# DeepMed-Lab-ECNU/BCP

Hardware: AMD Instinct MI355X
Metric: training volumes/sec (LA 112x112x80 V-Net, BCP self-training step) (higher is better)
Workload: dtype f32 (fp16x2 split operands); 1 GPU; LA 3D V-Net BCP self-train step, per-GPU batch 4 (2 labeled), 112x112x80 patches, SGD m0.9 wd1e-4, EMA 0.99 (BASELINE.json configs[1]); global_batch=4, parallelism=dp1

## Files before the change

### bcp_amd/csrc/api.hip

```cpp
#include "common.h"
#include "../../include/bcp_hip.h"
#include <cstring>

namespace bcp {
static thread_local char g_err[512] = "";
void set_error(const char* fmt, ...) {
  va_list ap;
  va_start(ap, fmt);
  vsnprintf(g_err, sizeof(g_err), fmt, ap);
  va_end(ap);
}
Options& options() {
  static Options o;
  return o;
}
}

extern "C" int bcp_version(void) { return BCP_ABI_VERSION; }

extern "C" int bcp_set_option(const char* name, const char* value) {
  BCP_REQUIRE(name && value, "bcp_set_option: null argument");
  bcp::Options& o = bcp::options();
  const bcp::Options def;
  long long v[5] = {0, 0, 0, 0, 0};
  const int n = sscanf(value, "%lld,%lld,%lld,%lld,%lld", &v[0], &v[1], &v[2], &v[3], &v[4]);
  const bool reset = n <= 0;
#define BCP_OPT_INT(field) if (!strcmp(name, #field)) { o.field = reset ? def.field : (int)v[0]; return BCP_OK; }
  BCP_OPT_INT(conv3_p) BCP_OPT_INT(splitk) BCP_OPT_INT(conv3_b6_flat_sk) BCP_OPT_INT(conv3_b6_cfg2d) BCP_OPT_INT(conv3_b6_w22) BCP_OPT_INT(conv3_b6_pipe) BCP_OPT_INT(conv3_b6_cin16max) BCP_OPT_INT(res_pcu) BCP_OPT_INT(res_nt) BCP_OPT_INT(wgrad_nt)
  BCP_OPT_INT(tn_groups) BCP_OPT_INT(cc_tile) BCP_OPT_INT(pack_sections) BCP_OPT_INT(cc_select_blocks) BCP_OPT_INT(conv3_b6) BCP_OPT_INT(conv3_b6_levels) BCP_OPT_INT(conv3_b6_direct) BCP_OPT_INT(conv3_b6_flat) BCP_OPT_INT(conv3_b6_minvox) BCP_OPT_INT(wgrad_b6) BCP_OPT_INT(wgrad_b6_minvox) BCP_OPT_INT(wgrad_b6_levels) BCP_OPT_INT(wgrad_b6_slots) BCP_OPT_INT(cc_border_dedupe) BCP_OPT_INT(cc_count_tile) BCP_OPT_INT(cc_fuse_select) BCP_OPT_INT(gemm_walk) BCP_OPT_INT(gemm_pipe) BCP_OPT_INT(gemm_stat_r) BCP_OPT_INT(norm_apply_cap) BCP_OPT_INT(norm_apply_vec) BCP_OPT_INT(k2_stats) BCP_OPT_INT(k2_bwd_stats) BCP_OPT_INT(up_recompute) BCP_OPT_INT(wgrad_b6_deep) BCP_OPT_INT(wgrad_b6_deep_nt) BCP_OPT_INT(wgrad_b6_deep_slots) BCP_OPT_INT(wgrad_b6_deep_tile) BCP_OPT_INT(norm_slabs) BCP_OPT_INT(conv3_f16) BCP_OPT_INT(fuse_bwd_stats) BCP_OPT_INT(conv3_xcd) BCP_OPT_INT(mix_c1) BCP_OPT_INT(whatif) BCP_OPT_INT(c3d16_form) BCP_OPT_INT(norm_own) BCP_OPT_INT(wgrad_reduce_flat) BCP_OPT_INT(norm_fin_rows) BCP_OPT_INT(norm_fuse_fin)
#undef BCP_OPT_INT
  if (!strcmp(name, "conv3_sk_elems")) { o.conv3_sk_elems = reset ? def.conv3_sk_elems : v[0]; return BCP_OK; }
  if (!strcmp(name, "res_tile2d_vox")) { o.res_tile2d_vox = reset ? def.res_tile2d_vox : v[0]; return BCP_OK; }
  if (!strcmp(name, "conv3_cfg")) {
    BCP_REQUIRE(reset || n == 4, "bcp_set_option: conv3_cfg wants TD,TH,TW,NT");
    for (int i = 0; i < 4; ++i) o.conv3_cfg[i] = reset ? 0 : (int)v[i];
    return BCP_OK;
  }
  if (!strcmp(name, "wgrad_tile")) {
    BCP_REQUIRE(reset || n >= 3, "bcp_set_option: wgrad_tile wants TD,TH,TW[,min_voxels,max_voxels]");
    for (int i = 0; i < 5; ++i) o.wgrad_tile[i] = def.wgrad_tile[i];
    for (int i = 0; i < n && !reset; ++i) o.wgrad_tile[i] = v[i];
    return BCP_OK;
  }
  bcp::set_error("bcp_set_option: unknown option '%s'", name);
  return BCP_EINVAL;
}
extern "C" const char* bcp_last_error(void) { return bcp::g_err; }

extern "C" int bcp_device_arch(char* buf, int n) {
  BCP_REQUIRE(buf && n > 0, "bcp_device_arch: bad buffer");
  int dev = 0;
  hipDeviceProp_t prop;
  if (hipGetDevice(&dev) != hipSuccess || hipGetDeviceProperties(&prop, dev) != hipSuccess) {
    bcp::set_error("bcp_device_arch: no HIP device");
    return BCP_ELAUNCH;
  }
  strncpy(buf, prop.gcnArchName, (size_t)n - 1);
  buf[n - 1] = 0;
  return BCP_OK;
}

extern "C" int bcp_event_create(void** ev) {
  BCP_REQUIRE(ev, "bcp_event_create: null");
  hipEvent_t e;
  if (hipEventCreate(&e) != hipSuccess) { bcp::set_error("hipEventCreate failed"); return BCP_ELAUNCH; }
  *ev = (void*)e;
  return BCP_OK;
}
extern "C" int bcp_event_record(void* ev, void* stream) {
  if (hipEventRecord((hipEvent_t)ev, (hipStream_t)stream) != hipSuccess) { bcp::set_error("hipEventRecord failed"); return BCP_ELAUNCH; }
  return BCP_OK;
}
extern "C" int bcp_event_elapsed_ms(void* start, void* stop, float* ms) {
  BCP_REQUIRE(ms, "bcp_event_elapsed_ms: null");
  if (hipEventSynchronize((hipEvent_t)stop) != hipSuccess || hipEventElapsedTime(ms, (hipEvent_t)start, (hipEvent_t)stop) != hipSuccess) {
    bcp::set_error("hipEventElapsedTime failed");
    return BCP_ELAUNCH;
  }
  return BCP_OK;
}
extern "C" int bcp_event_destroy(void* ev) {
  hipEventDestroy((hipEvent_t)ev);
// ... 36 lines not shown
```

### bcp_amd/csrc/common.h

```cpp
#pragma once
#include <hip/hip_runtime.h>
#include <cstdarg>
#include <cstdint>
#include <cstdio>

#define BCP_OK 0
#define BCP_EINVAL (-1)
#define BCP_ELAUNCH (-2)
#define BCP_EUNSUP (-3)

typedef float f32x4 __attribute__((ext_vector_type(4)));

namespace bcp {

void set_error(const char* fmt, ...);

#define BCP_REQUIRE(cond, ...)          \
  do {                                  \
    if (!(cond)) {                      \
      ::bcp::set_error(__VA_ARGS__);    \
      return BCP_EINVAL;                \
    }                                   \
  } while (0)

// ... 8 lines not shown

struct Options {
  int conv3_p = 0;
  int splitk = 0;
  long long conv3_sk_elems = 1LL << 20;
  int conv3_b6_cin16max = 32;
  int conv3_b6_pipe = 1;
  int conv3_b6_w22 = 1;
  int conv3_b6_cfg2d = 1;
  int conv3_b6_flat_sk = 0;
  int res_pcu = 0;
  int res_nt = 0;
  long long res_tile2d_vox = 10000;
  int conv3_cfg[4] = {0, 0, 0, 0};
  int wgrad_nt = 0;
  long long wgrad_tile[5] = {0, 0, 0, 0, 1LL << 60};
  int tn_groups = 0;
  int pack_sections = 7;
  int cc_tile = 0;
  int cc_select_blocks = 0;
  int conv3_b6 = 1;
  int conv3_b6_levels = 15;
  int conv3_b6_minvox = 256;
  int conv3_b6_flat = 1;
  int conv3_b6_direct = 1;
  int wgrad_b6 = 1;
  int wgrad_b6_minvox = 256;
  int norm_slabs = 1;
  int fuse_bwd_stats = 1;
  int conv3_xcd = 11;
  int conv3_f16 = 1;
  int wgrad_b6_slots = 0;
  int mix_c1 = 1;
  int wgrad_b6_deep = 1;
  int wgrad_b6_deep_nt = 0;
  int wgrad_b6_deep_slots = 0;
  int wgrad_b6_deep_tile = 1;
  int k2_stats = 2;
  int up_recompute = 0;
  int k2_bwd_stats = 0;
  int norm_fuse_fin = 1;
  int norm_fin_rows = 128;
  int gemm_pipe = 1;
  int gemm_stat_r = 0;
  int gemm_walk = 0;
  int cc_border_dedupe = 1;
  int cc_count_tile = 0;
  int cc_fuse_select = 1;
  int norm_apply_cap = 2048;
  int norm_apply_vec = 4;
  int wgrad_reduce_flat = 1;
  int norm_own = 0;
  int c3d16_form = 1;
  int whatif = 0;
  int wgrad_b6_levels = 15;
};
Options& options();

__device__ __forceinline__ unsigned char plabel_bin_of(float x0, float x1, float thres) {
  const float m = fmaxf(x0, x1);
  const float e0 = expf(x0 - m), e1 = expf(x1 - m);
  const float p1 = e1 / (e0 + e1);
  return (p1 >= thres) ? 1 : 0;
}
__device__ __forceinline__ unsigned char plabel_argmax4_of(float x0, float x1, float x2, float x3) {
  const float m = fmaxf(fmaxf(x0, x1), fmaxf(x2, x3));
  const float e0 = expf(x0 - m), e1 = expf(x1 - m), e2 = expf(x2 - m), e3 = expf(x3 - m);
  const float s = e0 + e1 + e2 + e3;
  const float p0 = e0 / s, p1 = e1 / s, p2 = e2 / s, p3 = e3 / s;
  int best = 0;
  float pb = p0;
  if (p1 > pb) { pb = p1; best = 1; }
  if (p2 > pb) { pb = p2; best = 2; }
  if (p3 > pb) { pb = p3; best = 3; }
  return (unsigned char)best;
}


static inline int cdiv(long long a, long long b) { return (int)((a + b - 1) / b); }
static inline bool aligned16(const void* p) { return (reinterpret_cast<uintptr_t>(p) & 15u) == 0; }

#ifndef BCP_LDS_BARRIER
#define BCP_LDS_BARRIER() asm volatile("s_waitcnt lgkmcnt(0)\n\ts_barrier" ::: "memory")
#endif

#ifndef BCP_GLDS16
typedef __attribute__((address_space(3))) void* bcp_lds_ptr_t;
#define BCP_GLDS16(gsrc, lds_wave_base) __builtin_amdgcn_global_load_lds((gsrc), (bcp_lds_ptr_t)(lds_wave_base), 16, 0, 0)
#define BCP_VM_LDS_BARRIER(N) asm volatile("s_waitcnt vmcnt(%0) lgkmcnt(0)\n\ts_barrier" ::"n"(N) : "memory")
#endif

#ifndef BCP_S_SLEEP
#define BCP_S_SLEEP(n) __builtin_amdgcn_s_sleep(n)
#endif

__device__ __forceinline__ float wave_sum(float v) {
#pragma unroll
  for (int o = 32; o > 0; o >>= 1) v += __shfl_xor(v, o);
  return v;
}
__device__ __forceinline__ double wave_sum(double v) {
#pragma unroll
  for (int o = 32; o > 0; o >>= 1) v += __shfl_xor(v, o);
  return v;
}

__device__ __forceinline__ unsigned long long wave_sum(unsigned long long v) {
#pragma unroll
  for (int o = 32; o > 0; o >>= 1) v += __shfl_xor(v, o);
  return v;
}

template <int NV>
__device__ __forceinline__ void block_sum_256(double (&v)[NV], double* lds ) {
  const int lane = threadIdx.x & 63, wid = threadIdx.x >> 6;
#pragma unroll
  for (int i = 0; i < NV; ++i) v[i] = wave_sum(v[i]);
  __syncthreads();
  if (lane == 0) {
#pragma unroll
    for (int i = 0; i < NV; ++i) lds[wid * NV + i] = v[i];
  }
  __syncthreads();
  if (threadIdx.x == 0) {
#pragma unroll
    for (int i = 0; i < NV; ++i) v[i] = lds[i] + lds[NV + i] + lds[2 * NV + i] + lds[3 * NV + i];
  }
}

constexpr int kAmaxSlots = 32, kAmaxStride = 32, kAmaxFloats = kAmaxSlots * kAmaxStride;
__device__ __forceinline__ void amax_clear(float* __restrict__ slots) {
  if (threadIdx.x < kAmaxSlots) slots[threadIdx.x * kAmaxStride] = 0.f;
}
__device__ __forceinline__ void block_amax_publish(float m, float* __restrict__ slots) {
  __shared__ float amax_red[4];
#pragma unroll
  for (int o = 32; o > 0; o >>= 1) { const float t = __shfl_xor(m, o); m = (t > m || t != t) ? t : m; }
  if ((threadIdx.x & 63) == 0) amax_red[threadIdx.x >> 6] = m;
  __syncthreads();
  if (threadIdx.x == 0) {
    for (int k = 1; k < 4; ++k) { const float t = amax_red[k]; m = (t > m || t != t) ? t : m; }
    if (m != m) m = __uint_as_float(0x7fc00000u);
    float* slot = slots + ((blockIdx.x + blockIdx.y * gridDim.x) % kAmaxSlots) * kAmaxStride;
    const float cur = __hip_atomic_load(slot, __ATOMIC_RELAXED, __HIP_MEMORY_SCOPE_AGENT);
// ... 40 lines not shown
```

### bcp_amd/csrc/conv3b.hip

```cpp
#include "conv3_defs.h"
#include "../../include/bcp_hip.h"

#ifndef B6_ABLATE
#define B6_ABLATE 0
#endif
#ifndef BCP_BW_ABLATE
#define BCP_BW_ABLATE 0
#endif
#ifndef BCP_C3D_STREAM
#define BCP_C3D_STREAM 1
#endif
#ifndef BCP_C3D_FD
#define BCP_C3D_FD 3
#endif
#ifndef BCP_C3D_MP
#define BCP_C3D_MP 2
#endif

#ifndef BCP_TS_DEBUG
#define BCP_TS_DEBUG 0
#endif
#if BCP_TS_DEBUG
__device__ unsigned long long bcp_ts_buf[64 * 64];
__device__ unsigned long long bcp_ts_span[8192 * 2];
// ... 640 lines not shown
    constexpr int tA = ((t0 / 9) * TL::HH + (t0 / 3) % 3) * TL::HW + t0 % 3, tB = ((t1 / 9) * TL::HH + (t1 / 3) % 3) * TL::HW + t1 % 3;
    const int toff = ((lg >> 1) ? tB : tA) * XSB;
    const unsigned short* Xc = Xb + NHB * XBUF + toff;
    const unsigned short* Wc = Wr + (sl1 >> 1) + woff;
    __builtin_amdgcn_sched_barrier(0);
    constexpr int NPR = PL * (PL + 1) / 2, NMEM = 5 * PL;
    constexpr int PI[6] = {PL == 3 ? 2 : 1, PL == 3 ? 1 : 0, 0, 1, 0, 0}, PJ[6] = {0, 1, PL == 3 ? 2 : 0, 0, 1, 0};
#pragma unroll
    for (int k = 0; k < 4 * NPR; ++k) {
      const int pr = k >> 2, mt = (k >> 1) & 1, nt = k & 1;
      acc[mt][nt] = PP::mfma(fb[PAR][nt][PJ[pr]], fa[PAR][mt][PI[pr]], acc[mt][nt]);
      if (k < PL) { if (dma_on) BCP_GLDS16(wst + wq[k < 3 ? k : 0], wdst + k * 4096); }
      else if (k < NMEM) {
        const int r = k - PL, sp = r >> 2, w = r & 3;
        if (w < 2) fa[PAR ^ 1][w][sp] = *reinterpret_cast<const frag_t*>(Xc + sp * XPLANE + voff[w]);
        else fb[PAR ^ 1][w - 2][sp] = *reinterpret_cast<const frag_t*>(Wc + sp * WPLANE + (w - 2) * 16 * 32);
      }
      if (k < NMEM) __builtin_amdgcn_sched_barrier(0);
    }
    __builtin_amdgcn_sched_barrier(0);
    if (dma_on) BCP_VM_LDS_BARRIER(PL); else BCP_VM_LDS_BARRIER(0);
    const unsigned t = sl0; sl0 = sl1; sl1 = sl2; sl2 = t;
    BCP_TS(3 + (cc - c_begin) * S + sg);
  };
  auto chunk = [&](int cc, auto hb_tag) __attribute__((always_inline)) {
#define BCP_ST(I) if constexpr (I < S) stage(cc, hb_tag, std::integral_constant<int, I>{});
    BCP_ST(0) BCP_ST(1) BCP_ST(2) BCP_ST(3) BCP_ST(4) BCP_ST(5) BCP_ST(6) BCP_ST(7) BCP_ST(8) BCP_ST(9) BCP_ST(10) BCP_ST(11) BCP_ST(12) BCP_ST(13)
#undef BCP_ST
  };
#pragma unroll 1
  for (int cc = c_begin; cc < c_end; cc += 2) {
    chunk(cc, std::integral_constant<int, 0>{});
    if (cc + 1 < c_end) chunk(cc + 1, std::integral_constant<int, 1>{});
  }
  BCP_TS(60);

  double s1[2][4], s2[2][4];
#pragma unroll
  for (int nt = 0; nt < 2; ++nt)
#pragma unroll
    for (int r = 0; r < 4; ++r) { s1[nt][r] = 0.0; s2[nt][r] = 0.0; }
  b6_store_tile<TL, TD, TH, TW, 2, 2, BW>(acc, Y, bias, cd, n, d0, h0, w0, cout0 + wn * 32, accumulate, st.partial != nullptr, s1, s2, wm, &st,
                                      st.partial ? bx / st.tiles_per_group : 0, osc);
  if (st.partial) {
    const int gg = bx / st.tiles_per_group, row = bx % st.tiles_per_group;
    BCP_LDS_BARRIER();
    stats_flush_22(s1, s2, Ss, st.partial + ((long long)gg * st.rows + row) * st.C * 2, cout0, cd.Cout);
  }
  BCP_TS(61);
  BCP_TSR(62);
}

#ifndef BCP_C3D_ATTR
#define BCP_C3D_ATTR
#endif
template <int KD, int TD, int TH, int TW, int NT, bool PER, bool BW = false, int PL = 3, bool WL = false>
__global__ __launch_bounds__(256) BCP_C3D_ATTR void k_c3d(const float* __restrict__ X, const float* __restrict__ Wp, const float* __restrict__ bias,
                                             float* __restrict__ Y, ConvDims cd, int n_tiles, int accumulate, StatsArg st) {
  using TL = Tile<KD, TD, TH, TW>;
  constexpr int MT = TL::MT, T = TL::T, TP = (T + 1) / 2, TPE = (TP + 1) & ~1, CT = NT * 16;
  constexpr int XPLANE = TL::HV * XSB;
  using HF = HaloFetch<TL>;
  using PP = Pipe<PL>;
  using frag_t = typename PP::frag;
  static_assert(!WL || (PER && NT == 1 && !BW), "LDS-resident weights: the persistent one-n-tile instances");

  BCP_TS(0);
  BCP_TSR(59);
  HIP_DYNAMIC_SHARED(float4, smem4)
  unsigned short* Xb = reinterpret_cast<unsigned short*>(smem4);
  double* Ss = reinterpret_cast<double*>(Xb + PL * XPLANE);
  frag_t* Wf = reinterpret_cast<frag_t*>(Ss + 4 * CT * 2);

  const int lane = threadIdx.x & 63;
  const int li = lane & 15, lg = lane >> 4, wave = threadIdx.x >> 6;
  const int cout0 = blockIdx.y * CT;

  int voff[MT];
#pragma unroll
  for (int mt = 0; mt < MT; ++mt) voff[mt] = TL::voff((wave * MT + mt) * 16 + b6_row<TW>(li)) * XSB + (lg & 1) * 8;
  HF hf;
  hf.init(cd, reinterpret_cast<float*>(smem4));

  f32x4 acc[MT][NT];
#pragma unroll
  for (int mt = 0; mt < MT; ++mt)
#pragma unroll
    for (int nt = 0; nt < NT; ++nt) acc[mt][nt] = (f32x4){0.f, 0.f, 0.f, 0.f};

  const int nchunks = cd.Cin16 >> 4;
  const int c_begin = (int)((long long)nchunks * blockIdx.z / gridDim.z), c_end = (int)((long long)nchunks * (blockIdx.z + 1) / gridDim.z);
  const int nch = c_end - c_begin;
  Y += (long long)blockIdx.z * cd.N * cd.D * cd.H * cd.W * cd.Cout;

  int t_first, t_step, my_tiles;
  if (!PER) {
    t_first = cd.xcd ? xcd_tile(blockIdx.x, gridDim.x, gridDim.x * (blockIdx.y + gridDim.y * blockIdx.z)) : (int)blockIdx.x;
    t_step = 0; my_tiles = 1;
  } else if ((cd.xcd & 2) && (gridDim.x & 7) == 0) {
    const int xc = blockIdx.x & 7, xs = (int)((long long)n_tiles * xc / 8), xe = (int)((long long)n_tiles * (xc + 1) / 8);
    t_step = gridDim.x >> 3;
    t_first = xs + (int)(blockIdx.x >> 3);
    my_tiles = t_first < xe ? (xe - 1 - t_first) / t_step + 1 : 0;
  } else {
    t_first = blockIdx.x; t_step = gridDim.x;
    my_tiles = (int)blockIdx.x < n_tiles ? (n_tiles - 1 - (int)blockIdx.x) / (int)gridDim.x + 1 : 0;
  }
  const int n_items = my_tiles * nch;

  const bool want_stats = PER && st.partial != nullptr;
  if (want_stats && (int)threadIdx.x < CT && cout0 + (int)threadIdx.x < cd.Cout) {
    for (int g = 0; g < st.G; ++g) {
      double* z = st.partial + (((long long)g * st.rows + blockIdx.x) * st.C + cout0 + threadIdx.x) * 2;
      z[0] = 0.0; z[1] = 0.0;
    }
  }
  if (n_items == 0) return;
  double s1[NT][4], s2[NT][4];
#pragma unroll
  for (int nt = 0; nt < NT; ++nt)
#pragma unroll
    for (int r = 0; r < 4; ++r) { s1[nt][r] = 0.0; s2[nt][r] = 0.0; }

  float xsc = 1.f, osc = 1.f;
  if (PL == 2) {
    const int ex = f16_scale_exp(amax_read(cd.xamax)), ew = f16_scale_exp(Wp[pack_off_hdr(T, cd.Cin16, cd.Cout16)]);
    xsc = ldexpf(1.f, ex);
    osc = ldexpf(1.f, -(ex + ew));
  }
  const unsigned short* Wl = reinterpret_cast<const unsigned short*>(Wp + PP::pack_off(T, cd.Cin16, cd.Cout16)) + (long long)(cout0 + li) * 32 + lg * 8;
  const long long piece_stride = (long long)cd.Cout16 * 32;
  auto bload = [&](int cc, int tp, frag_t (&b)[NT][PL]) __attribute__((always_inline)) {
    if (B6_ABLATE & 4) return;
    if constexpr (WL) {
#pragma unroll
      for (int s = 0; s < PL; ++s) b[0][s] = Wf[((tp < TP ? tp : TP - 1) * PL + s) * 64 + lane];
      return;
    }
    const unsigned short* p = Wl + ((long long)cc * TP + (tp < TP ? tp : TP - 1)) * PL * piece_stride;
#pragma unroll
    for (int s = 0; s < PL; ++s)
#pragma unroll
      for (int nt = 0; nt < NT; ++nt) b[nt][s] = *reinterpret_cast<const frag_t*>(p + s * piece_stride + nt * 16 * 32);
  };
  unsigned hvm = 0;
  float4 hpre[HF::NP];
  auto hfetch_item = [&](int it) __attribute__((always_inline)) {
    if (B6_ABLATE & 2) return;
    const int itc = it < n_items ? it : n_items - 1;
    const int tl = t_first + (itc / nch) * t_step;
    int n, d0, h0, w0;
    tile_origin(cd, tl, TD, TH, TW, n, d0, h0, w0);
    hvm = hf.fetch_nb(X, cd, n, d0, h0, w0, c_begin + itc % nch, hpre);
  };
  auto hstash = [&]() __attribute__((always_inline)) {
    if (B6_ABLATE & 2) return;
#pragma unroll
    for (int u = 0; u < HF::NP; ++u)
      if (hf.act && u * HF::RPP + hf.r0 < HF::HR) {
        const float4 v = ((hvm >> u) & 1u) ? hpre[u] : make_float4(0.f, 0.f, 0.f, 0.f);
        PP::split(v, xsc, Xb + ((u * HF::RPP + hf.r0) * TL::HW + hf.hw) * XSB + hf.part * 4, XPLANE);
      }
  };

  frag_t B0[NT][PL], B1[NT][PL];
  if (B6_ABLATE & 4) {
#pragma unroll
    for (int s = 0; s < PL; ++s)
#pragma unroll
      for (int nt = 0; nt < NT; ++nt) { B0[nt][s] = *reinterpret_cast<const frag_t*>(Xb + s * 64 + nt * 8 + lane); B1[nt][s] = B0[nt][s]; }
  }
  BCP_TS(1);
  if constexpr (WL) {
    const unsigned short* Wg = reinterpret_cast<const unsigned short*>(Wp + PP::pack_off(T, cd.Cin16, cd.Cout16)) + (long long)cout0 * 32;
    for (int i = threadIdx.x; i < TP * PL * 64; i += 256) {
      const int l = i & 63, f = i >> 6;
      Wf[i] = *reinterpret_cast<const frag_t*>(Wg + (long long)f * piece_stride + (l & 15) * 32 + (l >> 4) * 8);
    }
  }
  hfetch_item(0);
  if (!WL) bload(c_begin, 0, B0);
  hstash();
  BCP_LDS_BARRIER();
  if (WL) bload(c_begin, 0, B0);
  BCP_TS(2);
#ifndef BCP_C3D_HPF
#define BCP_C3D_HPF 3
#endif
  constexpr int HPF = TPE >= 10 ? (BCP_C3D_HPF >= 0 && !BW ? BCP_C3D_HPF : TPE - 6) : (TPE >= 6 ? TPE - 4 : 0);
  int cur_g = want_stats ? t_first / st.tiles_per_group : 0;
#pragma unroll 1
  for (int it = 0; it < n_items; ++it) {
    if (it > 0) {
      BCP_LDS_BARRIER();
      hstash();
      BCP_LDS_BARRIER();
    }
    const int cc = c_begin + it % nch;
    const int ccn = c_begin + (it + 1 < n_items ? (it + 1) % nch : it % nch);
#if BCP_C3D_STREAM
    frag_t nx[BCP_C3D_FD];
#endif
#pragma unroll
    for (int tp = 0; tp < TPE; ++tp) {
      if (tp & 1) { if (tp + 1 < TPE) bload(cc, tp + 1, B0); else bload(ccn, 0, B0); }
      else bload(cc, tp + 1, B1);
      if (tp == HPF) hfetch_item(it + 1);
      if (tp < TP && !(B6_ABLATE & 8)) {
        const int t0 = 2 * tp, t1 = 2 * tp + 1 < T ? 2 * tp + 1 : T - 1;
        const int tA = ((t0 / 9) * TL::HH + (t0 / 3) % 3) * TL::HW + t0 % 3, tB = ((t1 / 9) * TL::HH + (t1 / 3) % 3) * TL::HW + t1 % 3;
        const int toff = ((lg >> 1) ? tB : tA) * XSB;
#if BCP_C3D_STREAM
        {
          constexpr int MP = (NT > 1 && MT % BCP_C3D_MP == 0) ? BCP_C3D_MP : 1;
          constexpr int NF = MT * PL, FD = BCP_C3D_FD < NF ? BCP_C3D_FD : NF;
          static_assert(FD <= NF && MT % MP == 0, "fragment stream geometry");
          auto fidx = [&](int f, int& mt, int& I) __attribute__((always_inline)) { const int g = f / (PL * MP), r = f % (PL * MP); I = PL - 1 - r / MP; mt = g * MP + r % MP; };
          const int t0n = 2 * (tp + 1), t1n = 2 * (tp + 1) + 1 < T ? 2 * (tp + 1) + 1 : T - 1;
          const int tAn = ((t0n / 9) * TL::HH + (t0n / 3) % 3) * TL::HW + t0n % 3, tBn = ((t1n / 9) * TL::HH + (t1n / 3) % 3) * TL::HW + t1n % 3;
          const int toffn = ((lg >> 1) ? tBn : tAn) * XSB;
          const bool have_nx = tp > 0;
          const bool want_nx = tp + 1 < TP;
          frag_t fr[NF];
#pragma unroll
          for (int f = 0; f < FD; ++f) {
            int mt, I;
            fidx(f, mt, I);
            if (have_nx) fr[f] = nx[f];
            else fr[f] = *reinterpret_cast<const frag_t*>(Xb + I * XPLANE + voff[mt] + ((B6_ABLATE & 32) ? 0 : toff));
          }
#pragma unroll
          for (int f0 = 0; f0 < NF; f0 += MP) {
#pragma unroll
            for (int q = 0; q < MP; ++q) {
              const int g = f0 + q + FD;
              int mt, I;
              if (g < NF) { fidx(g, mt, I); fr[g] = *reinterpret_cast<const frag_t*>(Xb + I * XPLANE + voff[mt] + ((B6_ABLATE & 32) ? 0 : toff)); }
              else if (want_nx) { fidx(g - NF, mt, I); nx[g - NF] = *reinterpret_cast<const frag_t*>(Xb + I * XPLANE + voff[mt] + ((B6_ABLATE & 32) ? 0 : toffn)); }
            }
            __builtin_amdgcn_sched_barrier(0);
            int mt0, I;
            fidx(f0, mt0, I);
#pragma unroll
            for (int J = PL - 1 - I; J >= 0; --J)
#pragma unroll
              for (int q = 0; q < MP; ++q)
#pragma unroll
                for (int nt = 0; nt < NT; ++nt) {
                  if (tp & 1) acc[mt0 + q][nt] = PP::mfma(B1[nt][J], fr[f0 + q], acc[mt0 + q][nt]);
                  else acc[mt0 + q][nt] = PP::mfma(B0[nt][J], fr[f0 + q], acc[mt0 + q][nt]);
                }
            __builtin_amdgcn_sched_barrier(0);
          }
        }
#else
        static_assert(PL == 3, "the unstreamed tap loop exists for the bf16 planes only");
        bf16x8 a[MT][3];
#pragma unroll
        for (int s = 0; s < 3; ++s)
#pragma unroll
          for (int mt = 0; mt < MT; ++mt) a[mt][s] = *reinterpret_cast<const bf16x8*>(Xb + s * XPLANE + voff[mt] + ((B6_ABLATE & 32) ? 0 : toff));
#define BCP_B6(BS, I, J)                                                                                        \
  _Pragma("unroll") for (int mt = 0; mt < MT; ++mt) _Pragma("unroll") for (int nt = 0; nt < NT; ++nt)            \
      acc[mt][nt] = __builtin_amdgcn_mfma_f32_16x16x32_bf16(BS[nt][J], a[mt][I], acc[mt][nt], 0, 0, 0);
        if (tp & 1) { BCP_B6(B1, 2, 0) BCP_B6(B1, 1, 1) BCP_B6(B1, 0, 2) BCP_B6(B1, 1, 0) BCP_B6(B1, 0, 1) BCP_B6(B1, 0, 0) }
        else { BCP_B6(B0, 2, 0) BCP_B6(B0, 1, 1) BCP_B6(B0, 0, 2) BCP_B6(B0, 1, 0) BCP_B6(B0, 0, 1) BCP_B6(B0, 0, 0) }
#undef BCP_B6
#endif
      }
      if (!PER) BCP_TS(3 + it * TPE + tp);
    }
    if (it % nch == nch - 1) {
      const int tl = t_first + (it / nch) * t_step;
      int n, d0, h0, w0;
      tile_origin(cd, tl, TD, TH, TW, n, d0, h0, w0);
      if (!PER) {
        BCP_TS(60);
        BCP_LDS_BARRIER();
        b6_epilogue<TL, TD, TH, TW, NT, BW>(acc, Y, bias, cd, n, d0, h0, w0, cout0, accumulate, st, Ss, t_first, osc);
        BCP_TS(61);
        BCP_TSR(62);
        return;
      }
      if (want_stats && tl / st.tiles_per_group != cur_g) {
        BCP_LDS_BARRIER();
        stats_flush_t<NT>(s1, s2, Ss, st.partial + ((long long)cur_g * st.rows + blockIdx.x) * st.C * 2, cout0, cd.Cout);
        cur_g = tl / st.tiles_per_group;
      }
      b6_store_tile<TL, TD, TH, TW, NT, TL::MT, BW>(acc, Y, bias, cd, n, d0, h0, w0, cout0, accumulate, want_stats, s1, s2, -1, &st, cur_g, osc);
#pragma unroll
      for (int mt = 0; mt < MT; ++mt)
#pragma unroll
        for (int nt = 0; nt < NT; ++nt) acc[mt][nt] = (f32x4){0.f, 0.f, 0.f, 0.f};
    }
  }
  if (want_stats) {
    BCP_LDS_BARRIER();
    stats_flush_t<NT>(s1, s2, Ss, st.partial + ((long long)cur_g * st.rows + blockIdx.x) * st.C * 2, cout0, cd.Cout);
  }
}

template <int KD, int NT, int SP, int AVMAX>
__global__ __launch_bounds__(256) void k_c3f(const float* __restrict__ X, const float* __restrict__ Wp, const float* __restrict__ bias,
                                             float* __restrict__ Y, ConvDims cd, int tiles_per_sample, int accumulate, StatsArg st) {
  constexpr int BM = 64, T = KD * 9, TP = (T + 1) / 2, CT = NT * 16, PD = KD == 3 ? 1 : 0;
  constexpr int S = ((TP + SP - 1) / SP + 1) & ~1;
  static_assert(S >= 4, "the stage pipeline needs four weight stages per chunk");
  constexpr int XPLANE = AVMAX * XSB;
  constexpr int WPLANE = SP * CT * 32;
  constexpr int WSTAGE = 3 * WPLANE;
  constexpr int NW4 = (SP * 12 * CT + 255) / 256;
  constexpr int NP = (AVMAX * 4 + 255) / 256;

  HIP_DYNAMIC_SHARED(float4, smem4)
  unsigned short* Xb = reinterpret_cast<unsigned short*>(smem4);
  unsigned short* Wb = Xb + 3 * XPLANE;
  double* Ss = reinterpret_cast<double*>(Wb + 2 * WSTAGE);

  BCP_TS(0);
  BCP_TSR(59);
  const int lane = threadIdx.x & 63, wave = threadIdx.x >> 6;
  const int li = lane & 15, lg = lane >> 4;
  const int V = cd.D * cd.H * cd.W, HW = cd.H * cd.W;
  const int R = PD * HW + cd.W + 1, AV = BM + 2 * R;
  const int bx = cd.xcd ? xcd_tile(blockIdx.x, gridDim.x, gridDim.x * (blockIdx.y + gridDim.y * blockIdx.z)) : (int)blockIdx.x;
  const int n = bx / tiles_per_sample, m0 = (bx % tiles_per_sample) * BM;
  const int cout0 = blockIdx.y * CT;

  const int ml = wave * 16 + li, mv = m0 + ml;
  const int vrow = (ml + R) * XSB + (lg & 1) * 8;
  unsigned vbits = 0;
  {
    const int w = mv % cd.W, h = (mv / cd.W) % cd.H, d = mv / HW;
#pragma unroll
    for (int t = 0; t < T; ++t) {
      const int kw = t % 3, kh = (t / 3) % 3, kd = t / 9;
      const bool ok = (unsigned)(w + kw - 1) < (unsigned)cd.W && (unsigned)(h + kh - 1) < (unsigned)cd.H && (unsigned)(d + kd - PD) < (unsigned)cd.D;
      vbits |= (ok ? 1u : 0u) << t;
    }
    if (mv >= V) vbits = 0;
  }
  const int woff = li * 32 + ((lg ^ ((li & 8) ? 2 : 0)) * 8);
// ... 367 lines not shown
  const bool want_stats = st.partial != nullptr;
  if (mv < V) {
    float* yrow = Y + ((long long)n * V + mv) * cd.Cout + cout0 + lg * 4;
#pragma unroll
    for (int nt = 0; nt < NT; ++nt) {
#pragma unroll
      for (int r = 0; r < 4; ++r) {
        const int co = cout0 + nt * 16 + lg * 4 + r;
        float v = acc[nt][r] * osc + ((bias && co < cd.Cout) ? bias[co] : 0.f);
        if (accumulate && co < cd.Cout) v += yrow[nt * 16 + r];
        acc[nt][r] = v;
        if (want_stats && co < cd.Cout) { s1[nt][r] += (double)v; s2[nt][r] += (double)v * (double)v; }
      }
      if (vec) st4(yrow + nt * 16, make_float4(acc[nt][0], acc[nt][1], acc[nt][2], acc[nt][3]));
      else {
#pragma unroll
        for (int r = 0; r < 4; ++r)
          if (cout0 + nt * 16 + lg * 4 + r < cd.Cout) yrow[nt * 16 + r] = acc[nt][r];
      }
    }
  }
  if (want_stats) {
    const int gg = bx / st.tiles_per_group, row = bx % st.tiles_per_group;
    BCP_LDS_BARRIER();
    stats_flush_t<NT>(s1, s2, Ss, st.partial + ((long long)gg * st.rows + row) * st.C * 2, cout0, cd.Cout);
  }
  BCP_TS(61);
  BCP_TSR(62);
}

__global__ __launch_bounds__(256) void k_b6_sum_slabs(const float* __restrict__ part, int K, long long n, int Cout,
                                                      const float* __restrict__ bias, float* __restrict__ y, int accumulate) {
  for (long long i = (long long)blockIdx.x * blockDim.x + threadIdx.x; i < n; i += (long long)gridDim.x * blockDim.x) {
    float v = bias ? bias[i % Cout] : 0.f;
    for (int k = 0; k < K; ++k) v += part[(long long)k * n + i];
    y[i] = accumulate ? y[i] + v : v;
  }
}

template <int KD, int TD, int TH, int TW, int NT, int SP>
constexpr bool b6_has_bw() {
  return (KD == 3 && TD == 4 && TH == 8 && TW == 8 && NT == 2 && SP == 1) || (KD == 3 && TD == 4 && TH == 4 && TW == 8 && NT == 2 && SP == 1) ||
         (KD == 3 && TD == 4 && TH == 4 && TW == 4 && NT == 4 && SP == 1) || (KD == 1 && TD == 1 && TH == 16 && TW == 16 && NT == 2 && SP == 1) ||
         (KD == 1 && TD == 1 && TH == 8 && TW == 16 && NT == 2 && SP == 2);
}

template <int KD, int TD, int TH, int TW, int NT, int SP>
constexpr bool b6_has_f16() {
  return SP == 1 && ((KD == 3 && TD == 4 && TH == 8 && TW == 8 && (NT == 1 || NT == 2)) || (KD == 3 && TD == 4 && TH == 4 && TW == 8 && NT == 2) ||
                     (KD == 1 && TD == 1 && TH == 16 && TW == 16 && (NT == 1 || NT == 2)) ||
                     (KD == 1 && TD == 1 && TH == 8 && TW == 16 && NT == 4) ||
                     (KD == 3 && TD * TH * TW == 64 && NT == 4));
}

template <class TL, int PL = 3>
static constexpr size_t kC3pLds = (size_t)2 * PL * TL::HV * XSB * 2 + (size_t)3 * PL * 64 * 32 * 2 + (size_t)4 * 32 * 2 * sizeof(double);

thread_local int g_b6_last_planes = 3;

template <int KD, int TD, int TH, int TW, int NT, int SP>
static int b6_launch(const float* X, const float* Wp, const float* bias, float* Y, ConvDims cd, int accumulate, float* ws,
                     double* stat_partial, int G, bool dry, hipStream_t s, int* raw_sk, const BwdStatsIn* bw) {
  using TL = Tile<KD, TD, TH, TW>;
  constexpr int CT = NT * 16;
  const bool direct = options().conv3_b6_direct != 0 && (options().conv3_b6_direct >= 2 || (TL::MT == 4 && NT <= 2));
  const bool pipe64 = TL::M == 64 && NT == 4 && SP == 1 && options().conv3_b6_w22 != 0 && options().conv3_b6_pipe != 0;
  const bool staged2d = KD == 1 && NT == 4;
  const bool use_f16 = b6_has_f16<KD, TD, TH, TW, NT, SP>() && (staged2d || (NT == 4 ? pipe64 : direct)) && cd.xamax != nullptr && options().conv3_f16 != 0;
  if (!use_f16) cd.xamax = nullptr;
  const int npl = use_f16 ? 2 : 3;
  g_b6_last_planes = npl;
  const size_t lds = (size_t)npl * TL::HV * XSB * 2 + (direct ? 0 : (size_t)2 * npl * SP * CT * 32 * 2) + (size_t)4 * CT * 2 * sizeof(double);
  cd.tiles_d = cdiv(cd.D, TD); cd.tiles_h = cdiv(cd.H, TH); cd.tiles_w = cdiv(cd.W, TW);
  auto kfn = k_c3b<KD, TD, TH, TW, NT, SP>;
  if constexpr (KD == 1 && NT == 4 && b6_has_f16<KD, TD, TH, TW, NT, SP>()) {
    if (use_f16) kfn = k_c3b<KD, TD, TH, TW, NT, SP, false, 2>;
  }
  if (lds > 48 * 1024) hipFuncSetAttribute(reinterpret_cast<const void*>(kfn), hipFuncAttributeMaxDynamicSharedMemorySize, (int)lds);
  const int gx = cd.N * cd.tiles_d * cd.tiles_h * cd.tiles_w, gy = cd.Cout16 / CT;
  const int nch = cd.Cin16 / 16;
  int sk = 1;
  const bool ws_fits = ws && (long long)cd.N * cd.D * cd.H * cd.W * cd.Cout <= options().conv3_sk_elems;
  if (ws_fits && (long long)gx * gy <= 256 && nch >= 4) { sk = nch / 2; if (sk > 4) sk = 4; }
  { const int f = options().splitk; if (ws_fits && f >= 1 && f <= 4 && f <= nch) sk = f; }
  if (raw_sk) {
    *raw_sk = sk;
    if (dry) return 0;
    StatsArg none{nullptr, 0, 1, cd.Cout, 1};
    if (direct && NT != 1) {
      auto kd = k_c3d<KD, TD, TH, TW, NT, false>;
      if constexpr (b6_has_f16<KD, TD, TH, TW, NT, SP>()) {
        if (use_f16) kd = k_c3d<KD, TD, TH, TW, NT, false, false, 2>;
      }
      hipFuncSetAttribute(reinterpret_cast<const void*>(kd), hipFuncAttributeMaxDynamicSharedMemorySize, (int)lds);
      hipLaunchKernelGGL(kd, dim3(gx, gy, sk), dim3(256), lds, s, X, Wp, (const float*)nullptr, Y, cd, gx, 0, none);
    } else {
      size_t lds_k = lds + (direct ? (size_t)2 * npl * SP * CT * 32 * 2 : 0);
      if constexpr (TL::M == 64 && NT == 4 && SP == 1) {
        if (options().conv3_b6_w22 != 0) kfn = k_c3h<KD, TD, TH, TW>;
        if (options().conv3_b6_w22 != 0 && options().conv3_b6_pipe != 0) {
          kfn = k_c3p<KD, TD, TH, TW>; lds_k = kC3pLds<TL>;
          if constexpr (b6_has_f16<KD, TD, TH, TW, NT, SP>()) {
            if (use_f16) { kfn = k_c3p<KD, TD, TH, TW, false, 2>; lds_k = kC3pLds<TL, 2>; }
          }
        }
      }
      if (lds_k > 48 * 1024) hipFuncSetAttribute(reinterpret_cast<const void*>(kfn), hipFuncAttributeMaxDynamicSharedMemorySize, (int)lds_k);
      hipLaunchKernelGGL(kfn, dim3(gx, gy, sk), dim3(256), lds_k, s, X, Wp, (const float*)nullptr, Y, cd, 0, none);
    }
    return 0;
  }
  StatsArg st{nullptr, 0, 1, cd.Cout, G > 0 ? G : 1};
  if (sk == 1 && G > 0 && gx % G == 0) { st.rows = gx / G; st.tiles_per_group = gx / G; st.partial = stat_partial; }
  if (bw) {
    if (!b6_has_bw<KD, TD, TH, TW, NT, SP>() || sk != 1 || G <= 0 || gx % G || (direct && NT == 1)) return 0;
    if (options().fuse_bwd_stats == 2 && KD == 3 && NT == 2) return 0;
    st.by = bw->y; st.bstats = bw->stats; st.bact = bw->act;
  }
  if (direct) {
    constexpr bool PER = NT == 1;
    const int slots = 512 / (gy * sk) > 0 ? 512 / (gy * sk) : 1;
    const int per = PER ? cdiv(gx, slots) : 1;
    int P = cdiv(gx, per);
    if (PER && (cd.xcd & 2) && P >= 8) P = (P + 7) & ~7;
    if (PER && options().conv3_p > 0 && options().conv3_p < P) P = options().conv3_p;
    StatsArg sd{nullptr, 0, 1, cd.Cout, G > 0 ? G : 1};
    if (sk == 1 && G > 0 && gx % G == 0) { sd.rows = PER ? P : gx / G; sd.tiles_per_group = gx / G; sd.partial = stat_partial; }
    if (bw) { sd.by = bw->y; sd.bstats = bw->stats; sd.bact = bw->act; }
    if (dry) return (sk == 1 && G > 0 && gx % G == 0) ? (PER ? P : gx / G) : 0;
    auto kd = k_c3d<KD, TD, TH, TW, NT, PER>;
    if constexpr (b6_has_bw<KD, TD, TH, TW, NT, SP>() && !PER) {
      if (bw) kd = k_c3d<KD, TD, TH, TW, NT, PER, true>;
    }
    size_t lds_d = lds;
    if constexpr (b6_has_f16<KD, TD, TH, TW, NT, SP>()) {
      if (use_f16) {
        kd = k_c3d<KD, TD, TH, TW, NT, PER, false, 2>;
        if constexpr (b6_has_bw<KD, TD, TH, TW, NT, SP>() && !PER) {
          if (bw) kd = k_c3d<KD, TD, TH, TW, NT, PER, true, 2>;
        }
        if constexpr (PER) {
          if (options().c3d16_form != 0 && cd.Cin16 == 16 && sk == 1) {
            kd = k_c3d<KD, TD, TH, TW, NT, PER, false, 2, true>;
            lds_d += (size_t)((TL::T + 1) / 2) * 2 * 64 * 16;
          }
        }
      }
    }
    hipFuncSetAttribute(reinterpret_cast<const void*>(kd), hipFuncAttributeMaxDynamicSharedMemorySize, (int)lds_d);
    if (sk == 1) {
      hipLaunchKernelGGL(kd, dim3(P, gy, 1), dim3(256), lds_d, s, X, Wp, bias, Y, cd, gx, accumulate, sd);
    } else {
      const long long n = (long long)cd.N * cd.D * cd.H * cd.W * cd.Cout;
      StatsArg none{nullptr, 0, 1, cd.Cout, 1};
      hipLaunchKernelGGL(kd, dim3(P, gy, sk), dim3(256), lds_d, s, X, Wp, (const float*)nullptr, ws, cd, gx, 0, none);
      hipLaunchKernelGGL(k_b6_sum_slabs, dim3((int)((n + 255) / 256 > 1024 ? 1024 : (n + 255) / 256)), dim3(256), 0, s, ws, sk, n, cd.Cout, bias, Y,
                         accumulate);
    }
    return sd.partial ? sd.rows : 0;
  }
  if (dry) return sk == 1 && G > 0 && gx % G == 0 ? gx / G : 0;
  if constexpr (b6_has_bw<KD, TD, TH, TW, NT, SP>()) {
    if (bw) {
      kfn = k_c3b<KD, TD, TH, TW, NT, SP, true>;
      if (lds > 48 * 1024) hipFuncSetAttribute(reinterpret_cast<const void*>(kfn), hipFuncAttributeMaxDynamicSharedMemorySize, (int)lds);
    }
  }
  size_t lds_k = lds;
  if constexpr (TL::M == 64 && NT == 4 && SP == 1) {
    if (options().conv3_b6_w22 != 0) {
      kfn = k_c3h<KD, TD, TH, TW>;
      if constexpr (b6_has_bw<KD, TD, TH, TW, NT, SP>()) {
        if (bw) kfn = k_c3h<KD, TD, TH, TW, true>;
      }
      if (options().conv3_b6_pipe != 0) {
        kfn = k_c3p<KD, TD, TH, TW>;
        if constexpr (b6_has_bw<KD, TD, TH, TW, NT, SP>()) {
          if (bw) kfn = k_c3p<KD, TD, TH, TW, true>;
        }
        lds_k = kC3pLds<TL>;
        if constexpr (b6_has_f16<KD, TD, TH, TW, NT, SP>()) {
          if (use_f16) {
            kfn = k_c3p<KD, TD, TH, TW, false, 2>;
            if constexpr (b6_has_bw<KD, TD, TH, TW, NT, SP>()) {
              if (bw) kfn = k_c3p<KD, TD, TH, TW, true, 2>;
            }
            lds_k = kC3pLds<TL, 2>;
          }
        }
      }
      if (lds_k > 48 * 1024) hipFuncSetAttribute(reinterpret_cast<const void*>(kfn), hipFuncAttributeMaxDynamicSharedMemorySize, (int)lds_k);
    }
// ... 136 lines not shown
```

Baseline: 828.9 volumes/s.

## Add persistent two-n-tile direct conv3 form for 4x8x8 tiles with per-tile stats

Adds a persistent variant of the direct 3D conv kernel for the KD=3, 4x8x8, NT=2 fp16-split configuration. Each block now loops over several spatial tiles instead of one block per tile, and it writes statistics per tile rather than per group. Fragment addressing uses four precomputed tap-distance offsets, and opaque asm barriers keep the compiler from hoisting registers. The kernel also gets waves_per_eu hints. The aim is to cut launch and tail overhead and to improve LDS reuse, at the cost of more register pressure and a different stats-partial layout.

```diff
diff --git a/bcp_amd/csrc/api.hip b/bcp_amd/csrc/api.hip
--- a/bcp_amd/csrc/api.hip
+++ b/bcp_amd/csrc/api.hip
@@ -27,7 +27,7 @@
   const bool reset = n <= 0;
 #define BCP_OPT_INT(field) if (!strcmp(name, #field)) { o.field = reset ? def.field : (int)v[0]; return BCP_OK; }
   BCP_OPT_INT(conv3_p) BCP_OPT_INT(splitk) BCP_OPT_INT(conv3_b6_flat_sk) BCP_OPT_INT(conv3_b6_cfg2d) BCP_OPT_INT(conv3_b6_w22) BCP_OPT_INT(conv3_b6_pipe) BCP_OPT_INT(conv3_b6_cin16max) BCP_OPT_INT(res_pcu) BCP_OPT_INT(res_nt) BCP_OPT_INT(wgrad_nt)
-  BCP_OPT_INT(tn_groups) BCP_OPT_INT(cc_tile) BCP_OPT_INT(pack_sections) BCP_OPT_INT(cc_select_blocks) BCP_OPT_INT(conv3_b6) BCP_OPT_INT(conv3_b6_levels) BCP_OPT_INT(conv3_b6_direct) BCP_OPT_INT(conv3_b6_flat) BCP_OPT_INT(conv3_b6_minvox) BCP_OPT_INT(wgrad_b6) BCP_OPT_INT(wgrad_b6_minvox) BCP_OPT_INT(wgrad_b6_levels) BCP_OPT_INT(wgrad_b6_slots) BCP_OPT_INT(cc_border_dedupe) BCP_OPT_INT(cc_count_tile) BCP_OPT_INT(cc_fuse_select) BCP_OPT_INT(gemm_walk) BCP_OPT_INT(gemm_pipe) BCP_OPT_INT(gemm_stat_r) BCP_OPT_INT(norm_apply_cap) BCP_OPT_INT(norm_apply_vec) BCP_OPT_INT(k2_stats) BCP_OPT_INT(k2_bwd_stats) BCP_OPT_INT(up_recompute) BCP_OPT_INT(wgrad_b6_deep) BCP_OPT_INT(wgrad_b6_deep_nt) BCP_OPT_INT(wgrad_b6_deep_slots) BCP_OPT_INT(wgrad_b6_deep_tile) BCP_OPT_INT(norm_slabs) BCP_OPT_INT(conv3_f16) BCP_OPT_INT(fuse_bwd_stats) BCP_OPT_INT(conv3_xcd) BCP_OPT_INT(mix_c1) BCP_OPT_INT(whatif) BCP_OPT_INT(c3d16_form) BCP_OPT_INT(norm_own) BCP_OPT_INT(wgrad_reduce_flat) BCP_OPT_INT(norm_fin_rows) BCP_OPT_INT(norm_fuse_fin)
+  BCP_OPT_INT(tn_groups) BCP_OPT_INT(cc_tile) BCP_OPT_INT(pack_sections) BCP_OPT_INT(cc_select_blocks) BCP_OPT_INT(conv3_b6) BCP_OPT_INT(conv3_b6_levels) BCP_OPT_INT(conv3_b6_direct) BCP_OPT_INT(conv3_b6_flat) BCP_OPT_INT(conv3_b6_minvox) BCP_OPT_INT(wgrad_b6) BCP_OPT_INT(wgrad_b6_minvox) BCP_OPT_INT(wgrad_b6_levels) BCP_OPT_INT(wgrad_b6_slots) BCP_OPT_INT(cc_border_dedupe) BCP_OPT_INT(cc_count_tile) BCP_OPT_INT(cc_fuse_select) BCP_OPT_INT(gemm_walk) BCP_OPT_INT(gemm_pipe) BCP_OPT_INT(gemm_stat_r) BCP_OPT_INT(norm_apply_cap) BCP_OPT_INT(norm_apply_vec) BCP_OPT_INT(k2_stats) BCP_OPT_INT(k2_bwd_stats) BCP_OPT_INT(up_recompute) BCP_OPT_INT(wgrad_b6_deep) BCP_OPT_INT(wgrad_b6_deep_nt) BCP_OPT_INT(wgrad_b6_deep_slots) BCP_OPT_INT(wgrad_b6_deep_tile) BCP_OPT_INT(norm_slabs) BCP_OPT_INT(conv3_f16) BCP_OPT_INT(fuse_bwd_stats) BCP_OPT_INT(conv3_xcd) BCP_OPT_INT(mix_c1) BCP_OPT_INT(whatif) BCP_OPT_INT(c3d16_form) BCP_OPT_INT(c3d32_form) BCP_OPT_INT(norm_own) BCP_OPT_INT(wgrad_reduce_flat) BCP_OPT_INT(norm_fin_rows) BCP_OPT_INT(norm_fuse_fin)
 #undef BCP_OPT_INT
   if (!strcmp(name, "conv3_sk_elems")) { o.conv3_sk_elems = reset ? def.conv3_sk_elems : v[0]; return BCP_OK; }
   if (!strcmp(name, "res_tile2d_vox")) { o.res_tile2d_vox = reset ? def.res_tile2d_vox : v[0]; return BCP_OK; }
diff --git a/bcp_amd/csrc/common.h b/bcp_amd/csrc/common.h
--- a/bcp_amd/csrc/common.h
+++ b/bcp_amd/csrc/common.h
@@ -84,6 +84,7 @@
   int wgrad_reduce_flat = 1;
   int norm_own = 0;
   int c3d16_form = 1;
+  int c3d32_form = 1;
   int whatif = 0;
   int wgrad_b6_levels = 15;
 };
@@ -122,6 +123,16 @@
 #define BCP_VM_LDS_BARRIER(N) asm volatile("s_waitcnt vmcnt(%0) lgkmcnt(0)\n\ts_barrier" ::"n"(N) : "memory")
 #endif
 
+#ifndef BCP_OPAQUE_S
+#if defined(__AMDGCN__)
+#define BCP_OPAQUE_S(x) asm volatile("" : "+s"(x))
+#define BCP_OPAQUE_V(x) asm volatile("" : "+v"(x))
+#else
+#define BCP_OPAQUE_S(x) ((void)0)
+#define BCP_OPAQUE_V(x) ((void)0)
+#endif
+#endif
+
 #ifndef BCP_S_SLEEP
 #define BCP_S_SLEEP(n) __builtin_amdgcn_s_sleep(n)
 #endif
diff --git a/bcp_amd/csrc/conv3b.hip b/bcp_amd/csrc/conv3b.hip
--- a/bcp_amd/csrc/conv3b.hip
+++ b/bcp_amd/csrc/conv3b.hip
@@ -716,7 +716,11 @@
 }
 
 #ifndef BCP_C3D_ATTR
+#if defined(__HIP__)
+#define BCP_C3D_ATTR __attribute__((amdgpu_waves_per_eu((PER && NT > 1) ? 2 : 1)))
+#else
 #define BCP_C3D_ATTR
+#endif
 #endif
 template <int KD, int TD, int TH, int TW, int NT, bool PER, bool BW = false, int PL = 3, bool WL = false>
 __global__ __launch_bounds__(256) BCP_C3D_ATTR void k_c3d(const float* __restrict__ X, const float* __restrict__ Wp, const float* __restrict__ bias,
@@ -724,10 +728,11 @@
   using TL = Tile<KD, TD, TH, TW>;
   constexpr int MT = TL::MT, T = TL::T, TP = (T + 1) / 2, TPE = (TP + 1) & ~1, CT = NT * 16;
   constexpr int XPLANE = TL::HV * XSB;
-  using HF = HaloFetch<TL>;
+  using HF = HaloFetch<TL, (PER && NT > 1 && BW) ? XSB : XS>;
   using PP = Pipe<PL>;
   using frag_t = typename PP::frag;
   static_assert(!WL || (PER && NT == 1 && !BW), "LDS-resident weights: the persistent one-n-tile instances");
+  constexpr bool PT = PER && NT > 1;
 
   BCP_TS(0);
   BCP_TSR(59);
@@ -743,6 +748,20 @@
   int voff[MT];
 #pragma unroll
   for (int mt = 0; mt < MT; ++mt) voff[mt] = TL::voff((wave * MT + mt) * 16 + b6_row<TW>(li)) * XSB + (lg & 1) * 8;
+  constexpr int kTapDist[4] = {0, 1, TL::HW - 2, TL::HH * TL::HW - 2 * TL::HW - 2};
+  int vsel[PT ? 4 : 1][MT];
+  if constexpr (PT) {
+#pragma unroll
+    for (int c = 0; c < 4; ++c)
+#pragma unroll
+      for (int mt = 0; mt < MT; ++mt) vsel[c][mt] = voff[mt] + ((lg >> 1) ? kTapDist[c] * XSB : 0);
+  }
+  auto fptr = [&](int I, int mt, int tpq) __attribute__((always_inline)) -> const frag_t* {
+    const int t0 = 2 * tpq, t1 = 2 * tpq + 1 < T ? 2 * tpq + 1 : T - 1;
+    const int tA = ((t0 / 9) * TL::HH + (t0 / 3) % 3) * TL::HW + t0 % 3, tB = ((t1 / 9) * TL::HH + (t1 / 3) % 3) * TL::HW + t1 % 3;
+    const int dl = tB - tA, c = dl == kTapDist[0] ? 0 : dl == kTapDist[1] ? 1 : dl == kTapDist[2] ? 2 : 3;
+    return reinterpret_cast<const frag_t*>(Xb + I * XPLANE + ((B6_ABLATE & 32) ? 0 : tA * XSB) + vsel[(B6_ABLATE & 32) ? 0 : c][mt]);
+  };
   HF hf;
   hf.init(cd, reinterpret_cast<float*>(smem4));
 
@@ -772,7 +791,7 @@
   }
   const int n_items = my_tiles * nch;
 
-  const bool want_stats = PER && st.partial != nullptr;
+  const bool want_stats = PER && !PT && st.partial != nullptr;
   if (want_stats && (int)threadIdx.x < CT && cout0 + (int)threadIdx.x < cd.Cout) {
     for (int g = 0; g < st.G; ++g) {
       double* z = st.partial + (((long long)g * st.rows + blockIdx.x) * st.C + cout0 + threadIdx.x) * 2;
@@ -819,11 +838,14 @@
   };
   auto hstash = [&]() __attribute__((always_inline)) {
     if (B6_ABLATE & 2) return;
+    int slot = (hf.r0 * TL::HW + hf.hw) * XSB + hf.part * 4;
+    if constexpr (PT) BCP_OPAQUE_V(slot);
 #pragma unroll
     for (int u = 0; u < HF::NP; ++u)
       if (hf.act && u * HF::RPP + hf.r0 < HF::HR) {
         const float4 v = ((hvm >> u) & 1u) ? hpre[u] : make_float4(0.f, 0.f, 0.f, 0.f);
-        PP::split(v, xsc, Xb + ((u * HF::RPP + hf.r0) * TL::HW + hf.hw) * XSB + hf.part * 4, XPLANE);
+        if constexpr (PT) PP::split(v, xsc, Xb + u * HF::RPP * TL::HW * XSB + slot, XPLANE);
+        else PP::split(v, xsc, Xb + ((u * HF::RPP + hf.r0) * TL::HW + hf.hw) * XSB + hf.part * 4, XPLANE);
       }
   };
 
@@ -855,10 +877,24 @@
   int cur_g = want_stats ? t_first / st.tiles_per_group : 0;
 #pragma unroll 1
   for (int it = 0; it < n_items; ++it) {
+    if constexpr (PT && BW) {
+      int tid = threadIdx.x;
+      BCP_OPAQUE_V(tid);
+      hf.init(cd, reinterpret_cast<float*>(smem4), tid);
+    }
     if (it > 0) {
       BCP_LDS_BARRIER();
       hstash();
       BCP_LDS_BARRIER();
+    }
+    if constexpr (PT && BW) {
+#pragma unroll
+      for (int mt = 0; mt < MT; ++mt) {
+        int vo = voff[mt];
+        BCP_OPAQUE_V(vo);
+#pragma unroll
+        for (int c = 0; c < 4; ++c) vsel[c][mt] = vo + ((lg >> 1) ? kTapDist[c] * XSB : 0);
+      }
     }
     const int cc = c_begin + it % nch;
     const int ccn = c_begin + (it + 1 < n_items ? (it + 1) % nch : it % nch);
@@ -891,6 +927,7 @@
             int mt, I;
             fidx(f, mt, I);
             if (have_nx) fr[f] = nx[f];
+            else if constexpr (PT) fr[f] = *fptr(I, mt, tp);
             else fr[f] = *reinterpret_cast<const frag_t*>(Xb + I * XPLANE + voff[mt] + ((B6_ABLATE & 32) ? 0 : toff));
           }
 #pragma unroll
@@ -899,8 +936,8 @@
             for (int q = 0; q < MP; ++q) {
               const int g = f0 + q + FD;
               int mt, I;
-              if (g < NF) { fidx(g, mt, I); fr[g] = *reinterpret_cast<const frag_t*>(Xb + I * XPLANE + voff[mt] + ((B6_ABLATE & 32) ? 0 : toff)); }
-              else if (want_nx) { fidx(g - NF, mt, I); nx[g - NF] = *reinterpret_cast<const frag_t*>(Xb + I * XPLANE + voff[mt] + ((B6_ABLATE & 32) ? 0 : toffn)); }
+              if (g < NF) { fidx(g, mt, I); if constexpr (PT) fr[g] = *fptr(I, mt, tp); else fr[g] = *reinterpret_cast<const frag_t*>(Xb + I * XPLANE + voff[mt] + ((B6_ABLATE & 32) ? 0 : toff)); }
+              else if (want_nx) { fidx(g - NF, mt, I); if constexpr (PT) nx[g - NF] = *fptr(I, mt, tp + 1); else nx[g - NF] = *reinterpret_cast<const frag_t*>(Xb + I * XPLANE + voff[mt] + ((B6_ABLATE & 32) ? 0 : toffn)); }
             }
             __builtin_amdgcn_sched_barrier(0);
             int mt0, I;
@@ -946,12 +983,29 @@
         BCP_TSR(62);
         return;
       }
-      if (want_stats && tl / st.tiles_per_group != cur_g) {
-        BCP_LDS_BARRIER();
-        stats_flush_t<NT>(s1, s2, Ss, st.partial + ((long long)cur_g * st.rows + blockIdx.x) * st.C * 2, cout0, cd.Cout);
-        cur_g = tl / st.tiles_per_group;
-      }
-      b6_store_tile<TL, TD, TH, TW, NT, TL::MT, BW>(acc, Y, bias, cd, n, d0, h0, w0, cout0, accumulate, want_stats, s1, s2, -1, &st, cur_g, osc);
+      if constexpr (PT) {
+        int wv = __builtin_amdgcn_readfirstlane(wave), co0 = cout0;
+        BCP_OPAQUE_S(wv);
+        BCP_OPAQUE_S(co0);
+        const int gg = st.partial ? tl / st.tiles_per_group : 0;
+        double s1[NT][4], s2[NT][4];
+#pragma unroll
+        for (int nt = 0; nt < NT; ++nt)
+#pragma unroll
+          for (int r = 0; r < 4; ++r) { s1[nt][r] = 0.0; s2[nt][r] = 0.0; }
+        b6_store_tile<TL, TD, TH, TW, NT, TL::MT, BW>(acc, Y, bias, cd, n, d0, h0, w0, co0, accumulate, st.partial != nullptr, s1, s2, wv, &st, gg, osc);
+        if (st.partial) {
+          BCP_LDS_BARRIER();
+          stats_flush_t<NT>(s1, s2, Ss, st.partial + ((long long)gg * st.rows + tl % st.tiles_per_group) * st.C * 2, co0, cd.Cout);
+        }
+      } else {
+        if (want_stats && tl / st.tiles_per_group != cur_g) {
+          BCP_LDS_BARRIER();
+          stats_flush_t<NT>(s1, s2, Ss, st.partial + ((long long)cur_g * st.rows + blockIdx.x) * st.C * 2, cout0, cd.Cout);
+          cur_g = tl / st.tiles_per_group;
+        }
+        b6_store_tile<TL, TD, TH, TW, NT, TL::MT, BW>(acc, Y, bias, cd, n, d0, h0, w0, cout0, accumulate, want_stats, s1, s2, -1, &st, cur_g, osc);
+      }
 #pragma unroll
       for (int mt = 0; mt < MT; ++mt)
 #pragma unroll
@@ -1425,6 +1479,10 @@
                      (KD == 1 && TD == 1 && TH == 8 && TW == 16 && NT == 4) ||
                      (KD == 3 && TD * TH * TW == 64 && NT == 4));
 }
+
+template <int KD, int TD, int TH, int TW, int NT, int SP>
+constexpr bool b6_has_per32() { return SP == 1 && KD == 3 && TD == 4 && TH == 8 && TW == 8 && NT == 2; }
+static constexpr bool b6_per32_bw = true;
 
 template <class TL, int PL = 3>
 static constexpr size_t kC3pLds = (size_t)2 * PL * TL::HV * XSB * 2 + (size_t)3 * PL * 64 * 32 * 2 + (size_t)4 * 32 * 2 * sizeof(double);
@@ -1492,11 +1550,13 @@
   }
   if (direct) {
     constexpr bool PER = NT == 1;
+    bool PT = false;
+    if constexpr (b6_has_per32<KD, TD, TH, TW, NT, SP>()) PT = use_f16 && sk == 1 && options().c3d32_form != 0 && (!bw || b6_per32_bw);
     const int slots = 512 / (gy * sk) > 0 ? 512 / (gy * sk) : 1;
-    const int per = PER ? cdiv(gx, slots) : 1;
+    const int per = (PER || PT) ? cdiv(gx, slots) : 1;
     int P = cdiv(gx, per);
-    if (PER && (cd.xcd & 2) && P >= 8) P = (P + 7) & ~7;
-    if (PER && options().conv3_p > 0 && options().conv3_p < P) P = options().conv3_p;
+    if ((PER || PT) && (cd.xcd & 2) && P >= 8) P = (P + 7) & ~7;
+    if ((PER || PT) && options().conv3_p > 0 && options().conv3_p < P) P = options().conv3_p;
     StatsArg sd{nullptr, 0, 1, cd.Cout, G > 0 ? G : 1};
     if (sk == 1 && G > 0 && gx % G == 0) { sd.rows = PER ? P : gx / G; sd.tiles_per_group = gx / G; sd.partial = stat_partial; }
     if (bw) { sd.by = bw->y; sd.bstats = bw->stats; sd.bact = bw->act; }
@@ -1511,6 +1571,14 @@
         kd = k_c3d<KD, TD, TH, TW, NT, PER, false, 2>;
         if constexpr (b6_has_bw<KD, TD, TH, TW, NT, SP>() && !PER) {
           if (bw) kd = k_c3d<KD, TD, TH, TW, NT, PER, true, 2>;
+        }
+        if constexpr (b6_has_per32<KD, TD, TH, TW, NT, SP>()) {
+          if (PT) {
+            kd = k_c3d<KD, TD, TH, TW, NT, true, false, 2>;
+            if constexpr (b6_per32_bw && b6_has_bw<KD, TD, TH, TW, NT, SP>()) {
+              if (bw) kd = k_c3d<KD, TD, TH, TW, NT, true, true, 2>;
+            }
+          }
         }
         if constexpr (PER) {
           if (options().c3d16_form != 0 && cd.Cin16 == 16 && sk == 1) {
```

Result: faster. 839.4 volumes/s (median of 6 runs) (+1.3%).
